# sjtuytc/UnboundedNeRFPytorch

Measured on AMD Instinct MI355X. Metric: Msamples/sec (Mip-360 garden-shaped 1920x1080x256 frame, FourierGrid render), higher is better.
Workload: dtype f32; 1 GPU; S1 1920x1080x256 G200 F3(P7) C12 rgbnet 39-128-128-3 f32 stepsize 1.31 thres 1e-4 white-noise grids; rays=2073600, samples_per_ray=256, chunks_per_frame=1, parallelism=1 GPU, step=ray generation + march + shade + un-tiling to image order; 3 frames in flight

## Files before the change

### unboundednerfpytorch_amd/csrc/ugrid_march.hip

```cpp
#include "ugrid_render.h"
#include "ugrid_rays.h"

__global__ void k_pack_bricks(const float *__restrict__ grid, int P, int C, int X, int Y, int Z, int H,
                              int CH, int coef, float *__restrict__ out, int64_t total) {
  for (int64_t o = (int64_t)blockIdx.x * blockDim.x + threadIdx.x; o < total;
       o += (int64_t)gridDim.x * blockDim.x) {
    int64_t q = o;
    int ch, c;
    if (H == 2) {
      const int qi = (int)(q % (8 * CH)); q /= (8 * CH);
      c = (qi >> 1) & 7;
      ch = (qi >> 4) * 2 + (qi & 1);
    } else {
      ch = (int)(q % CH); q /= CH;
      c = (int)(q % 8); q /= 8;
    }
    const int h = (int)(q % H); q /= H;
    const int k = (int)(q % (Z - 1)); q /= (Z - 1);
    const int j = (int)(q % (Y - 1)); q /= (Y - 1);
    const int i = (int)(q % (X - 1)); q /= (X - 1);
    const int l = (int)q;
    const int chan = h * CH + ch;
    float v = 0.f;
    if (chan < C) {
// ... 812 lines not shown
  UG_LAUNCH_CHECK();
  return 0;
}

extern "C" int ugrid_train_sample_compact_vox(int64_t n_rays, int32_t slots_per_ray, float act_shift, float interval, float thres,
                                              const float *scratch_pts, const float *scratch_density, const int32_t *scratch_step,
                                              const float *scratch_w, const float *scratch_T, const int32_t *count,
                                              const int64_t *offset_end, const int32_t *count2, const int64_t *offset_end2,
                                              const float *t_table, float *pts1, float *density1, float *weights1, float *T1,
                                              int32_t *pos2, float *pts2, float *density2, float *alpha2, float *weights2,
                                              int64_t *ray_id2, int64_t *step_id2, float *t2, uint8_t *inner2, ugrid_stream_t s) {
  if (n_rays <= 0) return 0;
  hipLaunchKernelGGL(k_train_compact2, dim3(ug_blocks(n_rays * UG_WAVE, 256)), dim3(256), 0, ST(s), n_rays, slots_per_ray, act_shift,
                     interval, thres, scratch_pts, scratch_density, scratch_step, scratch_w, scratch_T, count, offset_end, count2,
                     offset_end2, t_table, pts1, density1, weights1, T1, pos2, pts2, density2, alpha2, weights2, ray_id2, step_id2, t2,
                     inner2, ug_tl_devn.cap > 0 ? ug_tl_devn.cap : INT64_MAX);
  UG_LAUNCH_CHECK();
  return 0;
}

extern "C" int ugrid_train_sample_backward(int64_t n_rays, float act_shift, float interval, const float *density1,
                                           const float *weights1, const float *T1, const int32_t *pos2, const int32_t *count,
                                           const int64_t *offset_end, const float *alphainv_last, const float *g_weights2,
                                           const float *g_alphainv_last, const float *g_density2, float *g_density1,
                                           ugrid_stream_t s) {
  if (n_rays <= 0) return 0;
  hipLaunchKernelGGL(k_train_sample_bwd, dim3(ug_blocks(n_rays * UG_WAVE, 256)), dim3(256), 0, ST(s), n_rays, act_shift, interval,
                     density1, weights1, T1, pos2, count, offset_end, alphainv_last, g_weights2, g_alphainv_last, g_density2, g_density1);
  UG_LAUNCH_CHECK();
  return 0;
}

extern "C" int ugrid_train_compact(int64_t n_rays, int32_t n_samples, const float *scratch_pts, const float *scratch_density,
                                   const int32_t *scratch_step, const int32_t *count, const int64_t *offset_end,
                                   const float *t_table, float *pts, float *density, int64_t *ray_id, int64_t *step_id,
                                   float *t, ugrid_stream_t s) {
  if (n_rays <= 0) return 0;
  hipLaunchKernelGGL(k_train_compact, dim3(ug_blocks(n_rays * UG_WAVE, 256)), dim3(256), 0, ST(s), n_rays, n_samples,
                     scratch_pts, scratch_density, scratch_step, count, offset_end, t_table, pts, density, ray_id, step_id, t);
  UG_LAUNCH_CHECK();
  return 0;
}

template <class MarchTile>
__device__ __forceinline__ void ug_march_block(const ug_ws_view &ws, int64_t nblocks, MarchTile march) {
  const int64_t blk = ug_xcd_remap(blockIdx.x, nblocks);
  if (blk >= nblocks) return;
  const int64_t tile = blk * 4 + (threadIdx.x >> 6);
  if (tile >= ws.n_tiles) return;
  const int n = march(tile, ws.ent + tile * ws.cap, ws.slot + tile * ws.cap);
  if (ug_lane() == 0) ws.count[tile] = n;
}

struct ug_march_geom { ug_ws_view ws; int64_t nblocks; dim3 grid; };
static inline ug_march_geom ug_march_geometry(void *ws_mem, int64_t n_rays, int32_t S) {
  ug_march_geom g;
  g.ws = ug_ws_make(ws_mem, n_rays, S);
  g.nblocks = (g.ws.n_tiles + 3) / 4;
  g.grid = dim3((unsigned)(((g.nblocks + 7) / 8) * 8));
  return g;
}

template <int F, bool L2, int W>
__global__ void __launch_bounds__(256, W)
k_march(ug_march_args a, const float *__restrict__ rays_o, const float *__restrict__ rays_d,
        const float *__restrict__ t_table, const float *__restrict__ s_table,
        const float *__restrict__ bricks, float *__restrict__ alphainv_last, float *__restrict__ depth,
        ug_ws_view ws, int64_t nblocks) {
  ug_march_block(ws, nblocks, [&](int64_t tile, float4 *ent, uint8_t *slot) {
    return ug_march_tile<F, L2>(a, rays_o, rays_d, t_table, s_table, bricks, alphainv_last, depth, tile, ent, slot);
  });
}


template <bool L2>
__global__ void __launch_bounds__(256, 5)
k_march_dcvgo(ug_march_args a, ug_dc_args dc, const float *__restrict__ rays_o, const float *__restrict__ rays_d,
              const float *__restrict__ t_table, const float *__restrict__ s_table, const float *__restrict__ bricks,
              float *__restrict__ alphainv_last, float *__restrict__ depth, float *__restrict__ wsum_mid, ug_ws_view ws,
              int64_t nblocks) {
  ug_march_block(ws, nblocks, [&](int64_t tile, float4 *ent, uint8_t *slot) {
    return ug_march_tile<0, L2, true>(a, rays_o, rays_d, t_table, s_table, bricks, alphainv_last, depth, tile, ent, slot, dc, wsum_mid);
  });
}

__global__ void __launch_bounds__(256, 6)
k_march_dvgo(ug_march_args a, ug_dv_args dv, const float *__restrict__ rays_o, const float *__restrict__ rays_d,
             const float *__restrict__ bricks, float *__restrict__ alphainv_last, float *__restrict__ depth, ug_ws_view ws,
             int64_t nblocks) {
  ug_march_block(ws, nblocks, [&](int64_t tile, float4 *ent, uint8_t *slot) {
    return ug_march_tile_dvgo(a, dv, rays_o, rays_d, bricks, alphainv_last, depth, tile, ent, slot, a.S);
  });
}

__global__ void __launch_bounds__(256, 6)
k_march_mpi(ug_march_args a, ug_mpi_args mp, const float *__restrict__ rays_o, const float *__restrict__ rays_d,
            const float *__restrict__ bricks, const float *__restrict__ act_shift, float *__restrict__ alphainv_last,
            float *__restrict__ depth, ug_ws_view ws, int64_t nblocks) {
  __shared__ float shift[256];
  if ((int)threadIdx.x < mp.D) shift[threadIdx.x] = act_shift[threadIdx.x];
  __syncthreads();
  ug_march_block(ws, nblocks, [&](int64_t tile, float4 *ent, uint8_t *slot) {
    return ug_march_tile_mpi(a, mp, rays_o, rays_d, bricks, shift, alphainv_last, depth, tile, ent, slot);
  });
}

extern "C" int64_t ugrid_render_ws_bytes(int64_t n_rays, int32_t S) {
  const int64_t n_tiles = (n_rays + UG_WAVE - 1) / UG_WAVE, cap = (int64_t)UG_WAVE * S;
  return 256 + ug_align256(n_tiles * 4) + ug_align256(n_tiles * cap * 16) + ug_align256(n_tiles * cap);
}

static int ug_grid_query_any(bool cl, const float *grid, int P, int C, int X, int Y, int Z, const float *xyz,
                             const float *xyz_min, const float *xyz_max, int freq_num, int64_t n, float *out, hipStream_t st) {
  if (n <= 0) return 0;
  if (P != (freq_num > 0 ? 2 * freq_num + 1 : 1)) return (int)hipErrorInvalidValue;
  const int64_t nl = ug_launch_rows(n);
  if (cl)
    hipLaunchKernelGGL(HIP_KERNEL_NAME(k_grid_query<true>), dim3(ug_blocks(nl * C, 256)), dim3(256), 0, st, grid, P, C, X, Y, Z, xyz,
                       xyz_min, xyz_max, freq_num, n, out, ug_tl_devn.ptr);
  else
    hipLaunchKernelGGL(HIP_KERNEL_NAME(k_grid_query<false>), dim3(ug_blocks(nl, 256)), dim3(256), 0, st, grid, P, C, X, Y, Z, xyz,
                       xyz_min, xyz_max, freq_num, n, out, ug_tl_devn.ptr);
  UG_LAUNCH_CHECK();
// ... 51 lines not shown
                                            int Z, float *acc, ugrid_stream_t s) {
  if (n_rays <= 0 || n_samples <= 0) return 0;
  if (!rays_o || !rays_d || !xyz_min || !xyz_max || !acc || X < 1 || Y < 1 || Z < 1) return (int)hipErrorInvalidValue;
  hipLaunchKernelGGL(k_count_views_accumulate, dim3(ug_blocks(n_rays, 64)), dim3(64), 0, ST(s), rays_o, rays_d, n_rays, xyz_min, xyz_max,
                     near, far, stepdist, n_samples, X, Y, Z, acc);
  UG_LAUNCH_CHECK();
  return 0;
}

extern "C" int ugrid_count_views_commit(float *acc, float *count, int64_t n, ugrid_stream_t s) {
  if (n <= 0) return 0;
  if (!acc || !count) return (int)hipErrorInvalidValue;
  const int64_t blocks = ug_blocks(n, 256);
  hipLaunchKernelGGL(k_count_views_commit, dim3((unsigned)(blocks < 65536 ? blocks : 65536)), dim3(256), 0, ST(s), acc, count, n);
  UG_LAUNCH_CHECK();
  return 0;
}

static inline int ug_brick_ch(int C, int *H) {
  if (C == 1) { *H = 1; return 1; }
  *H = 2;
  return UG_CH(C);
}

extern "C" int64_t ugrid_brick_bytes(int P, int C, int X, int Y, int Z, int direct) {
  int H, CH = ug_brick_ch(C, &H);
  if (direct) { H = 1; CH = 4; }
  return (int64_t)P * (X - 1) * (Y - 1) * (Z - 1) * H * 8 * CH * (int64_t)sizeof(float);
}

extern "C" int ugrid_pack_bricks(const float *grid, int P, int C, int X, int Y, int Z, int direct,
                                 float *bricks, ugrid_stream_t s) {
  if (X < 2 || Y < 2 || Z < 2 || P < 1 || C < 1) return (int)hipErrorInvalidValue;
  int H, CH = ug_brick_ch(C, &H);
  if (direct) { H = 1; CH = 4; }
  const int64_t total = (int64_t)P * (X - 1) * (Y - 1) * (Z - 1) * H * 8 * CH;
  int64_t blocks = (total + 255) / 256;
  if (blocks > 256 * 64) blocks = 256 * 64;
  if (C == 12 && !direct) {
    if (P > 1 && (int64_t)(X - 1) * (Y - 1) * (Z - 1) * 384 >= ((int64_t)1 << 32)) return (int)hipErrorInvalidValue;
    hipLaunchKernelGGL(k_pack_quad, dim3((unsigned)blocks), dim3(256), 0, ST(s), grid, P, C, X, Y, Z, bricks, total);
    UG_LAUNCH_CHECK();
    return 0;
  }
  int coef = direct ? 0 : 1;
  hipLaunchKernelGGL(k_pack_bricks, dim3((unsigned)blocks), dim3(256), 0, ST(s), grid, P, C, X, Y, Z, H, CH,
                     coef, bricks, total);
  UG_LAUNCH_CHECK();
  return 0;
}

static int g_march_waves = 6;
extern "C" int ug_set_march_waves(int w) { if (w < 4 || w > 6) return 1; g_march_waves = w; return 0; }

template <int F, int W>
static int ug_march_launch_w(const ugrid_render_params *p, const ug_march_args &a, const float *rays_o,
                             const float *rays_d, const float *t_table, const float *s_table,
                             const float *bricks, float *alphainv_last, float *depth, const ug_march_geom &g,
                             hipStream_t st) {
  if (p->norm_l2)
    hipLaunchKernelGGL(HIP_KERNEL_NAME(k_march<F, true, W>), g.grid, dim3(256), 0, st, a, rays_o,
                       rays_d, t_table, s_table, bricks, alphainv_last, depth, g.ws, g.nblocks);
  else
    hipLaunchKernelGGL(HIP_KERNEL_NAME(k_march<F, false, W>), g.grid, dim3(256), 0, st, a, rays_o,
                       rays_d, t_table, s_table, bricks, alphainv_last, depth, g.ws, g.nblocks);
  UG_LAUNCH_CHECK();
  return 0;
}

template <int F>
static int ug_march_launch(const ugrid_render_params *p, const ug_march_args &a, const float *rays_o,
                           const float *rays_d, const float *t_table, const float *s_table,
                           const float *bricks, float *alphainv_last, float *depth, const ug_march_geom &g,
                           hipStream_t st) {
  switch (g_march_waves) {
    case 4: return ug_march_launch_w<F, 4>(p, a, rays_o, rays_d, t_table, s_table, bricks, alphainv_last, depth, g, st);
    case 6: return ug_march_launch_w<F, 6>(p, a, rays_o, rays_d, t_table, s_table, bricks, alphainv_last, depth, g, st);
    default: return ug_march_launch_w<F, 5>(p, a, rays_o, rays_d, t_table, s_table, bricks, alphainv_last, depth, g, st);
  }
}

extern "C" int ugrid_render_march(const ugrid_render_params *p, const float *rays_o, const float *rays_d,
                                  const float *t_table, const float *s_table, const float *density_bricks,
                                  float *alphainv_last, float *depth, void *ws_mem, ugrid_stream_t s) {
  if (p->n_rays <= 0) return 0;
  ug_march_args a;
  const int rc = ug_fill_march_args(p, a);
  if (rc) return rc;
  const ug_march_geom g = ug_march_geometry(ws_mem, p->n_rays, p->n_samples);
  switch (p->freq_num) {
    case 1: return ug_march_launch<1>(p, a, rays_o, rays_d, t_table, s_table, density_bricks, alphainv_last, depth, g, ST(s));
    case 2: return ug_march_launch<2>(p, a, rays_o, rays_d, t_table, s_table, density_bricks, alphainv_last, depth, g, ST(s));
    case 3: return ug_march_launch<3>(p, a, rays_o, rays_d, t_table, s_table, density_bricks, alphainv_last, depth, g, ST(s));
    case 4: return ug_march_launch<4>(p, a, rays_o, rays_d, t_table, s_table, density_bricks, alphainv_last, depth, g, ST(s));
    case 5: return ug_march_launch<5>(p, a, rays_o, rays_d, t_table, s_table, density_bricks, alphainv_last, depth, g, ST(s));
    default: return (int)hipErrorInvalidValue;
  }
}


extern "C" int ugrid_render_march_dcvgo(const ugrid_render_params *p, const ugrid_dcvgo_params *q, const float *rays_o,
                                        const float *rays_d, const float *t_table, const float *s_table,
                                        const float *density_bricks, float *alphainv_last, float *depth, float *wsum_mid,
                                        void *ws_mem, ugrid_stream_t s) {
  if (p->n_rays <= 0) return 0;
  if (p->freq_num != 0 || !q) return (int)hipErrorInvalidValue;
  ug_march_args a;
  ug_dc_args dc;
  int rc = ug_fill_mask_args(dc, q->mask, q->mask_x, q->mask_y, q->mask_z, q->xyz2ijk_scale, q->xyz2ijk_shift);
  if (!rc) rc = ug_fill_march_args(p, a);
  if (rc) return rc;
  dc.dist_thres = q->dist_thres;
  const ug_march_geom g = ug_march_geometry(ws_mem, p->n_rays, p->n_samples);
  if (p->norm_l2)
    hipLaunchKernelGGL(HIP_KERNEL_NAME(k_march_dcvgo<true>), g.grid, dim3(256), 0, ST(s), a, dc, rays_o, rays_d, t_table,
                       s_table, density_bricks, alphainv_last, depth, wsum_mid, g.ws, g.nblocks);
  else
    hipLaunchKernelGGL(HIP_KERNEL_NAME(k_march_dcvgo<false>), g.grid, dim3(256), 0, ST(s), a, dc, rays_o, rays_d, t_table,
                       s_table, density_bricks, alphainv_last, depth, wsum_mid, g.ws, g.nblocks);
  UG_LAUNCH_CHECK();
// ... 43 lines not shown
```

### unboundednerfpytorch_amd/csrc/ugrid_render.h

```cpp
#pragma once
#include "ugrid_common.h"
#include "ugrid_math.h"
#include <string.h>

#define UG_CH(C) (2 * (((C) + 3) / 4))
#define UG_MAX_F 5


typedef float f32x16 __attribute__((ext_vector_type(16)));

struct ug_vec3 { float x, y, z; };

__device__ __forceinline__ float ug_norm3_torch(float x, float y, float z) {
  return sqrtf(fmaf(z, z, fmaf(y, y, x * x)));
}

template <bool L2>
__device__ __forceinline__ ug_vec3 ug_contract(ug_vec3 p, float B, float A) {
  const float nrm = L2 ? ug_norm3_torch(p.x, p.y, p.z) : fmaxf(fabsf(p.x), fmaxf(fabsf(p.y), fabsf(p.z)));
  if (!(nrm <= 1.0f)) {
    const float sc = B - (1.0f / nrm) * A;
    p.x = p.x / nrm * sc;
    p.y = p.y / nrm * sc;
    p.z = p.z / nrm * sc;
// ... 478 lines not shown
  }
#pragma unroll
  for (int s = 0; s < CH; ++s) feat[s] = 0.f;
#pragma unroll
  for (int b0 = 0; b0 < P; b0 += NB) {
    float4 v[NB][2 * CH];
#pragma unroll
    for (int l = 0; l < NB; ++l)
      if (b0 + l < P) {
#pragma unroll
        for (int q = 0; q < 2 * CH; ++q) v[l][q] = c[b0 + l].rec[q];
      }
    __builtin_amdgcn_sched_barrier(0);
#pragma unroll
    for (int l = 0; l < NB; ++l)
      if (b0 + l < P) {
        const float tz = c[b0 + l].tz, ty = c[b0 + l].ty, tx = c[b0 + l].tx;
#pragma unroll
        for (int pr = 0; pr < CH / 2; ++pr) {
          const float4 q0 = v[l][4 * pr], q1 = v[l][4 * pr + 1], q2 = v[l][4 * pr + 2], q3 = v[l][4 * pr + 3];
          const float a00 = fmaf(q0.z, tz, q0.x), a01 = fmaf(q1.z, tz, q1.x);
          const float a10 = fmaf(q2.z, tz, q2.x), a11 = fmaf(q3.z, tz, q3.x);
          const float b00 = fmaf(q0.w, tz, q0.y), b01 = fmaf(q1.w, tz, q1.y);
          const float b10 = fmaf(q2.w, tz, q2.y), b11 = fmaf(q3.w, tz, q3.y);
          const float fa = fmaf(fmaf(a11, ty, a10), tx, fmaf(a01, ty, a00));
          const float fb = fmaf(fmaf(b11, ty, b10), tx, fmaf(b01, ty, b00));
          feat[2 * pr] = (b0 + l == 0) ? fa : feat[2 * pr] + fa;
          feat[2 * pr + 1] = (b0 + l == 0) ? fb : feat[2 * pr + 1] + fb;
        }
      }
  }
#pragma unroll
  for (int ch = 0; ch < CH; ++ch) feat[ch] = ug_div_r(feat[ch], (float)P, 1.0f / (float)P);
}

typedef float ug_f4 __attribute__((ext_vector_type(4)));
template <int IMM>
__device__ __forceinline__ ug_f4 ug_gload4(unsigned voff, const float *sbase) {
  ug_f4 r;
  asm volatile("global_load_dwordx4 %0, %1, %2 offset:%3" : "=v"(r) : "v"(voff), "s"(sbase), "n"(IMM) : "memory");
  return r;
}
template <int IMM>
__device__ __forceinline__ ug_f4 ug_gload4v(const char *vaddr) {
  ug_f4 r;
  asm volatile("global_load_dwordx4 %0, %1, off offset:%2" : "=v"(r) : "v"(vaddr), "n"(IMM) : "memory");
  return r;
}
template <int N>
__device__ __forceinline__ void ug_vmwait6(ug_f4 (&v)[6]) {
  asm volatile("s_waitcnt vmcnt(%6)" : "+v"(v[0]), "+v"(v[1]), "+v"(v[2]), "+v"(v[3]), "+v"(v[4]), "+v"(v[5]) : "n"(N));
}

template <int K>
__device__ __forceinline__ float ug_quad_bcast(float x) {
  return __int_as_float(__builtin_amdgcn_mov_dpp(__float_as_int(x), K * 0x55, 0xf, 0xf, true));
}

__device__ __forceinline__ void ug_quad_poly(const ug_f4 (&v)[6], float tx, float ty, float tz, bool first, float (&feat)[3]) {
#pragma unroll
  for (int c = 0; c < 3; ++c) {
    const ug_f4 lo = v[2 * c], hi = v[2 * c + 1];
    const float p00 = fmaf(lo.y, tz, lo.x), p01 = fmaf(lo.w, tz, lo.z);
    const float p10 = fmaf(hi.y, tz, hi.x), p11 = fmaf(hi.w, tz, hi.z);
    const float f = fmaf(fmaf(p11, ty, p10), tx, fmaf(p01, ty, p00));
    feat[c] = first ? f : feat[c] + f;
  }
}

struct ug_quad_axis { float lo, ex, ir, nm1, nm2; unsigned goff; };
__device__ __forceinline__ ug_quad_axis ug_quad_axis_of(const ug_shade_args &a, int g) {
  ug_quad_axis q;
  q.lo = g == 0 ? a.lox : (g == 1 ? a.loy : a.loz);
  q.ex = g == 0 ? a.ex : (g == 1 ? a.ey : a.ez);
  q.ir = g == 0 ? a.irx : (g == 1 ? a.iry : a.irz);
  const int n = g == 0 ? a.X : (g == 1 ? a.Y : a.Z);
  q.nm1 = (float)(n - 1); q.nm2 = (float)(n - 2);
  q.goff = (unsigned)g * 16u;
  return q;
}

template <int F, int NBL, int NR>
struct ug_gather_state {
  static constexpr int P = 2 * F + 1, NI = NR * P;
  unsigned off[NI];
  float tx[NI], ty[NI], tz[NI];
  ug_f4 v[NBL][6];
};

#define UG_ISSUE_ITEM(st_, i_)                                                                                     \
  if constexpr (F == 0) {      \
    const char *pa = (const char *)k0b + (uint64_t)st_.off[i_] * 384ull + (uint64_t)((ug_lane() & 3) * 16);        \
    st_.v[(i_) % NBL][0] = ug_gload4v<0>(pa);   st_.v[(i_) % NBL][1] = ug_gload4v<64>(pa);                          \
    st_.v[(i_) % NBL][2] = ug_gload4v<128>(pa); st_.v[(i_) % NBL][3] = ug_gload4v<192>(pa);                         \
    st_.v[(i_) % NBL][4] = ug_gload4v<256>(pa); st_.v[(i_) % NBL][5] = ug_gload4v<320>(pa);                         \
  } else {                                                                                                         \
    const float *lb = k0b + (int64_t)((i_) / NR) * lvl_floats;                                                     \
    st_.v[(i_) % NBL][0] = ug_gload4<0>(st_.off[i_], lb);   st_.v[(i_) % NBL][1] = ug_gload4<64>(st_.off[i_], lb);  \
    st_.v[(i_) % NBL][2] = ug_gload4<128>(st_.off[i_], lb); st_.v[(i_) % NBL][3] = ug_gload4<192>(st_.off[i_], lb); \
    st_.v[(i_) % NBL][4] = ug_gload4<256>(st_.off[i_], lb); st_.v[(i_) % NBL][5] = ug_gload4<320>(st_.off[i_], lb); \
  }

template <int F, int NBL, int NR>
__device__ __forceinline__ void ug_k0_gather_begin(const float *__restrict__ k0b, const ug_shade_args &a,
                                                   const ug_quad_axis &qa, const float (&p_g)[NR],
                                                   ug_gather_state<F, NBL, NR> &st) {
// ... 910 lines not shown
```

### unboundednerfpytorch_amd/csrc/ugrid_shade.hip

```cpp
#include "ugrid_render.h"
#include "ugrid_shade_pc.h"

extern "C" int ug_set_march_waves(int w);
extern "C" int ug_set_tv_xcd(int m);
extern "C" int ug_set_train_mlp(int m);
#define UG_PC12_NBL 3
static int g_shade_pc = 2;

__global__ void k_pack_mlp(const float *__restrict__ w0, const float *__restrict__ b0,
                           const float *__restrict__ w1, const float *__restrict__ b1,
                           const float *__restrict__ w2, const float *__restrict__ b2, int C, int n_emb,
                           ug_mlp_scales sc, float *__restrict__ out) {
  const ug_mlp_layout L = ug_mlp_lay(C, n_emb);
  const int mlp_in = C + n_emb;
  unsigned short *hx = (unsigned short *)(out + L.hxA1);
  const int n_hx = (L.hxB1 - L.hxA1) * 2;
  for (int i = blockIdx.x * blockDim.x + threadIdx.x; i < n_hx; i += gridDim.x * blockDim.x) {
    const int e = i & 7, lane = (i >> 3) & 63, u = i >> 9;
    const int part = u & 1, o = (u >> 1) & 3, step = u >> 3;
    float w = 0.f;
    if (step < L.KB1) {
      const int idx = 8 * step + e;
      const int col = idx < L.KL ? ug_in_col(idx, lane >> 5, C, n_emb, L.KL) : -1;
      if (col >= 0) w = w0[(32 * o + (lane & 31)) * mlp_in + col] * sc.sW1;
    } else {
      const int st = step - L.KB1;
      w = w1[(32 * o + (lane & 31)) * 128 + ug_feat_of(st >> 1, 8 * (st & 1) + e, lane >> 5)] * sc.sW2;
    }
    const _Float16 hh = (_Float16)w;
    const _Float16 ll = (_Float16)(w - (float)hh);
    hx[i] = __builtin_bit_cast(unsigned short, part == 0 ? hh : ll);
  }
  if (blockIdx.x == 0 && threadIdx.x < 4)
    out[L.hxS + threadIdx.x] = threadIdx.x == 0 ? sc.sX1 : (threadIdx.x == 1 ? sc.sX2 / (sc.sW1 * sc.sX1) : 0.f);
  unsigned short *bf = (unsigned short *)(out + L.bfA1);
  const int n_bf = (L.bfB1 - L.bfA1) * 2;
  for (int i = blockIdx.x * blockDim.x + threadIdx.x; i < n_bf; i += gridDim.x * blockDim.x) {
    const int e = i & 7, lane = (i >> 3) & 63, u = i >> 9;
    const int part = u % 3, o = (u / 3) & 3, step = u / 12;
    float w = 0.f;
    if (step < L.KB1) {
      const int idx = 8 * step + e;
      const int col = idx < L.KL ? ug_in_col(idx, lane >> 5, C, n_emb, L.KL) : -1;
      if (col >= 0) w = w0[(32 * o + (lane & 31)) * mlp_in + col];
    } else {
      const int st = step - L.KB1;
      w = w1[(32 * o + (lane & 31)) * 128 + ug_feat_of(st >> 1, 8 * (st & 1) + e, lane >> 5)];
    }
    const __bf16 hh = (__bf16)w;
    const float r1 = w - (float)hh;
    const __bf16 mm = (__bf16)r1;
    const __bf16 ll = (__bf16)(r1 - (float)mm);
    const __bf16 pick = part == 0 ? hh : (part == 1 ? mm : ll);
    bf[i] = __builtin_bit_cast(unsigned short, pick);
  }
  for (int i = blockIdx.x * blockDim.x + threadIdx.x; i < L.total; i += gridDim.x * blockDim.x) {
// ... 146 lines not shown
      finite = finite && std::isfinite(a);
      m1 = a > m1 ? a : m1;
      acc += a * (k < C ? fb : 1.0);
    }
    finite = finite && std::isfinite(acc);
    B1 = acc > B1 ? acc : B1;
  }
  for (size_t i = 0; i < (size_t)128 * 128; ++i) {
    const double a = std::fabs((double)h_w1[i]);
    finite = finite && std::isfinite(a);
    m2 = a > m2 ? a : m2;
  }
  const double B0 = fb > 1.0 ? fb : 1.0;
  ug_mlp_scales sc = {1.f, 1.f, 1.f, 1.f};
  bool ok = finite && k0_absmax > 0 && std::isfinite(fb) && std::isfinite(B1) && std::isfinite(m1) && std::isfinite(m2) &&
            m1 > 1e-30 && m2 > 1e-30 && B1 > 1e-30;
  if (ok) {
    sc.sX1 = ug_pow2_floor(32768.0 / B0);
    sc.sW1 = ug_pow2_floor(32768.0 / m1);
    sc.sX2 = ug_pow2_floor(32768.0 / B1);
    sc.sW2 = ug_pow2_floor(32768.0 / m2);
    const float lo = 1.0f / 1024.0f, hi = 1099511627776.0f;
    ok = sc.sX1 >= lo && sc.sX2 >= lo && sc.sW1 >= lo && sc.sW2 >= lo && sc.sX1 <= hi && sc.sX2 <= hi &&
         sc.sW1 <= hi && sc.sW2 <= hi;
    if (!ok) sc = {1.f, 1.f, 1.f, 1.f};
  }
  scales4[0] = sc.sX1; scales4[1] = sc.sW1; scales4[2] = sc.sX2; scales4[3] = sc.sW2;
  return ok ? 1 : 0;
}

extern "C" int ugrid_pack_mlp(const float *w0, const float *b0, const float *w1, const float *b1,
                              const float *w2, const float *b2, int32_t k0_channels, int32_t viewbase_pe,
                              int32_t width, float k0_absmax, float *packed, int32_t *best_mode,
                              ugrid_stream_t s) {
  if (width != 128) return (int)hipErrorInvalidValue;
  const int C = k0_channels, n_emb = 3 + 6 * (int)viewbase_pe, mlp_in = C + n_emb;
  std::vector<float> h0((size_t)128 * mlp_in), hb0(128), h1((size_t)128 * 128);
  UG_HIP(hipMemcpyAsync(h0.data(), w0, h0.size() * sizeof(float), hipMemcpyDeviceToHost, ST(s)));
  UG_HIP(hipMemcpyAsync(hb0.data(), b0, hb0.size() * sizeof(float), hipMemcpyDeviceToHost, ST(s)));
  UG_HIP(hipMemcpyAsync(h1.data(), w1, h1.size() * sizeof(float), hipMemcpyDeviceToHost, ST(s)));
  UG_HIP(hipStreamSynchronize(ST(s)));
  float sc4[4];
  const int ok = ugrid_mlp_fp16x2_scales(h0.data(), hb0.data(), h1.data(), k0_channels, viewbase_pe, k0_absmax, sc4);
  const ug_mlp_scales sc = {sc4[0], sc4[1], sc4[2], sc4[3]};
  hipLaunchKernelGGL(k_pack_mlp, dim3(64), dim3(256), 0, ST(s), w0, b0, w1, b1, w2, b2, C, n_emb, sc, packed);
  UG_LAUNCH_CHECK();
  if (best_mode) *best_mode = (ok && viewbase_pe <= 4) ? UGRID_MLP_FP16X2 : UGRID_MLP_BF16X3;
  return 0;
}

extern "C" int ugrid_tune(const char *key, int value) {
  if (!key) return (int)hipErrorInvalidValue;
  if (!strcmp(key, "march_waves")) return ug_set_march_waves(value) ? (int)hipErrorInvalidValue : 0;
  if (!strcmp(key, "tv_xcd")) return ug_set_tv_xcd(value) ? (int)hipErrorInvalidValue : 0;
  if (!strcmp(key, "train_mlp")) return ug_set_train_mlp(value) ? (int)hipErrorInvalidValue : 0;
  if (!strcmp(key, "shade_pc") && value >= 0 && value <= 2) { g_shade_pc = value; return 0; }
  return (int)hipErrorInvalidValue;
}

template <int F, int C, int PE, int NW, int BF>
static int ug_shade_launch_nw(const ug_shade_args &a, const float *viewdirs, const float *k0b, const float *mlp,
                              ug_ws_view ws, float *rgb, int32_t *counter, hipStream_t st) {
  const int lds_bytes = ug_shade_lds_bytes<C, PE, BF, NW>();
  UG_SET_DYN_LDS((k_shade_mlp<F, C, PE, NW, BF>), lds_bytes);
  UG_ZERO_WORDS(counter, 8, st);
  int64_t wgs = (ws.n_tiles + NW - 1) / NW;
  if (wgs > 256) wgs = 256;
  wgs = (wgs + 7) / 8 * 8;
  hipLaunchKernelGGL(HIP_KERNEL_NAME(k_shade_mlp<F, C, PE, NW, BF>), dim3((unsigned)wgs), dim3(NW * 64), lds_bytes, st, a,
                     viewdirs, k0b, mlp, ws, rgb, counter);
  UG_LAUNCH_CHECK();
  return 0;
}


template <int F, int PE, int NPAIR, int SLOTS, int NBL, int MODE, bool ROLL = false>
static int ug_shade_pc_launch(const ug_shade_args &a, const float *viewdirs, const float *k0b, const float *mlp,
                              ug_ws_view ws, float *rgb, int32_t *counter, hipStream_t st) {
  const int lds_bytes = ug_pc_lds_bytes<PE, NPAIR, SLOTS>();
  if (lds_bytes > 160 * 1024) return (int)hipErrorInvalidValue;
  UG_SET_DYN_LDS((k_shade_pc<F, PE, NPAIR, SLOTS, NBL, MODE, ROLL>), lds_bytes);
  UG_ZERO_WORDS(counter, 8, st);
  int64_t wgs = (ws.n_tiles + NPAIR - 1) / NPAIR;
  if (wgs > 256) wgs = 256;
  wgs = (wgs + 7) / 8 * 8;
  hipLaunchKernelGGL(HIP_KERNEL_NAME(k_shade_pc<F, PE, NPAIR, SLOTS, NBL, MODE, ROLL>), dim3((unsigned)wgs), dim3(NPAIR * 128), lds_bytes, st,
                     a, viewdirs, k0b, mlp, ws, rgb, counter);
  UG_LAUNCH_CHECK();
  return 0;
}

template <int F, int C, int PE>
static int ug_shade_launch(const ug_shade_args &a, const float *viewdirs, const float *k0b, const float *mlp,
                           ug_ws_view ws, float *rgb, int32_t *counter, int mlp_mode, hipStream_t st) {
  if constexpr (PE > 4) {
    if (mlp_mode == UGRID_MLP_FP16X2) return (int)hipErrorInvalidValue;
  }
  if constexpr (C == 12 && PE <= 4) {
    if constexpr (F <= 3) {
      if (mlp_mode == UGRID_MLP_FP16X2 && g_shade_pc >= 2)
        return ug_shade_pc_launch<F, PE, 6, 2, UG_PC12_NBL, 1>(a, viewdirs, k0b, mlp, ws, rgb, counter, st);
    } else {
      if (mlp_mode == UGRID_MLP_FP16X2 && g_shade_pc >= 2)
        return ug_shade_pc_launch<F, PE, 6, 2, UG_PC12_NBL, 1, true>(a, viewdirs, k0b, mlp, ws, rgb, counter, st);
    }
    if (mlp_mode == UGRID_MLP_FP16X2 && g_shade_pc >= 1)
// ... 52 lines not shown
```

Measured before the change: 64940 Msamples/s.

## Add software-pipelined march kernel that prefetches brick loads across levels and samples

Adds a new march kernel, on by default, that uses a K-deep register ring of in-flight brick loads across the Fourier levels and issues the next sample's loads while the current sample's levels are still being consumed, using explicit vmcnt waits and scheduling barriers. Ray data and positions are staged in LDS, and t/s table values are read with scalar loads. The goal is to hide global memory latency in the density march. The cost is more registers and LDS per thread, which can lower occupancy, and a large amount of hand-scheduled inline asm that is fragile.

Measured after the change: 64030 Msamples/s. 0.986x the previous value.

```diff
diff --git a/unboundednerfpytorch_amd/csrc/ugrid_march.hip b/unboundednerfpytorch_amd/csrc/ugrid_march.hip
--- a/unboundednerfpytorch_amd/csrc/ugrid_march.hip
+++ b/unboundednerfpytorch_amd/csrc/ugrid_march.hip
@@ -888,6 +888,16 @@
   if (ug_lane() == 0) ws.count[tile] = n;
 }
 
+template <class MarchTile>
+__device__ __forceinline__ void ug_march_block_uniform(const ug_ws_view &ws, int64_t nblocks, MarchTile march) {
+  const int64_t blk = ug_xcd_remap(blockIdx.x, nblocks);
+  if (blk >= nblocks) return;
+  const int64_t tile = blk * 4 + __builtin_amdgcn_readfirstlane((int)(threadIdx.x >> 6));
+  if (tile >= ws.n_tiles) return;
+  const int n = march(tile, ws.ent + tile * ws.cap, ws.slot + tile * ws.cap);
+  if (ug_lane() == 0) ws.count[tile] = n;
+}
+
 struct ug_march_geom { ug_ws_view ws; int64_t nblocks; dim3 grid; };
 static inline ug_march_geom ug_march_geometry(void *ws_mem, int64_t n_rays, int32_t S) {
   ug_march_geom g;
@@ -905,6 +915,17 @@
         ug_ws_view ws, int64_t nblocks) {
   ug_march_block(ws, nblocks, [&](int64_t tile, float4 *ent, uint8_t *slot) {
     return ug_march_tile<F, L2>(a, rays_o, rays_d, t_table, s_table, bricks, alphainv_last, depth, tile, ent, slot);
+  });
+}
+
+template <int F, bool L2, int W>
+__global__ void __launch_bounds__(256, W)
+k_march_pipe(ug_march_args a, const float *__restrict__ rays_o, const float *__restrict__ rays_d,
+             const float *__restrict__ t_table, const float *__restrict__ s_table,
+             const float *__restrict__ bricks, float *__restrict__ alphainv_last, float *__restrict__ depth,
+             ug_ws_view ws, int64_t nblocks) {
+  ug_march_block_uniform(ws, nblocks, [&](int64_t tile, float4 *ent, uint8_t *slot) {
+    return ug_march_tile_pipe<F, L2>(a, rays_o, rays_d, t_table, s_table, bricks, alphainv_last, depth, tile, ent, slot);
   });
 }
 
@@ -1062,20 +1083,38 @@
 
 static int g_march_waves = 6;
 extern "C" int ug_set_march_waves(int w) { if (w < 4 || w > 6) return 1; g_march_waves = w; return 0; }
+static int g_march_pipe = 1;
+extern "C" int ug_set_march_pipe(int m) { if (m < 0 || m > 1) return 1; g_march_pipe = m; return 0; }
+
+template <int F, int W, bool PIPE>
+static int ug_march_launch_wp(const ugrid_render_params *p, const ug_march_args &a, const float *rays_o,
+                             const float *rays_d, const float *t_table, const float *s_table,
+                             const float *bricks, float *alphainv_last, float *depth, const ug_march_geom &g,
+                             hipStream_t st) {
+  if constexpr (PIPE) {
+    if (p->norm_l2)
+      hipLaunchKernelGGL(HIP_KERNEL_NAME(k_march_pipe<F, true, W>), g.grid, dim3(256), 0, st, a, rays_o,
+                         rays_d, t_table, s_table, bricks, alphainv_last, depth, g.ws, g.nblocks);
+    else
+      hipLaunchKernelGGL(HIP_KERNEL_NAME(k_march_pipe<F, false, W>), g.grid, dim3(256), 0, st, a, rays_o,
+                         rays_d, t_table, s_table, bricks, alphainv_last, depth, g.ws, g.nblocks);
+  } else if (p->norm_l2)
+    hipLaunchKernelGGL(HIP_KERNEL_NAME(k_march<F, true, W>), g.grid, dim3(256), 0, st, a, rays_o,
+                       rays_d, t_table, s_table, bricks, alphainv_last, depth, g.ws, g.nblocks);
+  else
+    hipLaunchKernelGGL(HIP_KERNEL_NAME(k_march<F, false, W>), g.grid, dim3(256), 0, st, a, rays_o,
+                       rays_d, t_table, s_table, bricks, alphainv_last, depth, g.ws, g.nblocks);
+  UG_LAUNCH_CHECK();
+  return 0;
+}
 
 template <int F, int W>
 static int ug_march_launch_w(const ugrid_render_params *p, const ug_march_args &a, const float *rays_o,
                              const float *rays_d, const float *t_table, const float *s_table,
                              const float *bricks, float *alphainv_last, float *depth, const ug_march_geom &g,
                              hipStream_t st) {
-  if (p->norm_l2)
-    hipLaunchKernelGGL(HIP_KERNEL_NAME(k_march<F, true, W>), g.grid, dim3(256), 0, st, a, rays_o,
-                       rays_d, t_table, s_table, bricks, alphainv_last, depth, g.ws, g.nblocks);
-  else
-    hipLaunchKernelGGL(HIP_KERNEL_NAME(k_march<F, false, W>), g.grid, dim3(256), 0, st, a, rays_o,
-                       rays_d, t_table, s_table, bricks, alphainv_last, depth, g.ws, g.nblocks);
-  UG_LAUNCH_CHECK();
-  return 0;
+  if (g_march_pipe) return ug_march_launch_wp<F, W, true>(p, a, rays_o, rays_d, t_table, s_table, bricks, alphainv_last, depth, g, st);
+  return ug_march_launch_wp<F, W, false>(p, a, rays_o, rays_d, t_table, s_table, bricks, alphainv_last, depth, g, st);
 }
 
 template <int F>
diff --git a/unboundednerfpytorch_amd/csrc/ugrid_render.h b/unboundednerfpytorch_amd/csrc/ugrid_render.h
--- a/unboundednerfpytorch_amd/csrc/ugrid_render.h
+++ b/unboundednerfpytorch_amd/csrc/ugrid_render.h
@@ -554,6 +554,238 @@
   asm volatile("s_waitcnt vmcnt(%6)" : "+v"(v[0]), "+v"(v[1]), "+v"(v[2]), "+v"(v[3]), "+v"(v[4]), "+v"(v[5]) : "n"(N));
 }
 
+template <int N>
+__device__ __forceinline__ void ug_vmwait2(ug_f4 &lo, ug_f4 &hi) {
+  asm volatile("s_waitcnt vmcnt(%2)" : "+v"(lo), "+v"(hi) : "n"(N));
+}
+
+#ifndef UG_MARCH_PIPE_K
+#define UG_MARCH_PIPE_K 4
+#endif
+constexpr int ug_mp_last(int P, int K, int s) { return s + K * ((P - 1 - s) / K); }
+constexpr int ug_mp_when(int P, int K, int s) {
+  int e = P - K - 1 > 0 ? P - K - 1 : 0;
+  for (int i = 0; i <= s; ++i) e = ug_mp_last(P, K, i) > e ? ug_mp_last(P, K, i) : e;
+  return e;
+}
+constexpr int ug_mp_after(int P, int K, int l) {
+  int n = (l + K - 1 < P - 1 ? l + K - 1 : P - 1) - l;
+  for (int s = 0; s < K; ++s) n += ug_mp_when(P, K, s) < l ? 1 : 0;
+  return n;
+}
+
+__device__ __forceinline__ float ug_sload(const float *p) {
+  float v;
+  asm volatile("s_load_dword %0, %1, 0x0" : "=s"(v) : "s"(p) : "memory");
+  return v;
+}
+__device__ __forceinline__ void ug_swait(float &v) { asm volatile("s_waitcnt lgkmcnt(0)" : "+s"(v)); }
+
+__device__ __forceinline__ float ug_uniformf(float v) {
+  return __uint_as_float(__builtin_amdgcn_readfirstlane(__float_as_uint(v)));
+}
+struct ug_mp_grid { float xm1, xm2, ym1, ym2, zm1, zm2; unsigned zrow, off_max; };
+__device__ __forceinline__ void ug_mp_axis(float c, float nm1, float nm2, float &cellf, float &whi) {
+  const float ix = fmaf(c, 0.5f, 0.5f) * nm1;
+  cellf = __builtin_amdgcn_fmed3f(floorf(ix), 0.0f, nm2);
+  whi = ix - cellf;
+}
+
+struct ug_mp_pt { float ux, uy, uz; };
+
+template <int K>
+struct ug_mp_ring {
+  ug_f4 lo[K], hi[K];
+  float tx[K], ty[K], tz[K];
+  float cx, cy, cz;
+};
+
+template <bool L2>
+__device__ __forceinline__ ug_mp_pt ug_mp_point(const ug_march_args &a, const float *ray_lds, float *pos_lds, float t) {
+  const float ox = ray_lds[0], oy = ray_lds[256], oz = ray_lds[512], dx = ray_lds[768], dy = ray_lds[1024], dz = ray_lds[1280];
+  float px = ox + dx * t, py = oy + dy * t, pz = oz + dz * t;
+  const float nrm = L2 ? ug_norm3_torch(px, py, pz) : fmaxf(fabsf(px), fmaxf(fabsf(py), fabsf(pz)));
+  if (!(nrm <= 1.0f)) {
+    const float rn = ug_rcp_refined(nrm);
+    const float sc = a.B - rn * a.A;
+    px = ug_div_r(px, nrm, rn) * sc;
+    py = ug_div_r(py, nrm, rn) * sc;
+    pz = ug_div_r(pz, nrm, rn) * sc;
+  }
+  ug_mp_pt q;
+  pos_lds[0] = px; pos_lds[256] = py; pos_lds[512] = pz;
+  ug_normalise(a, px, py, pz, q.ux, q.uy, q.uz);
+  return q;
+}
+
+template <int K, int L>
+__device__ __forceinline__ void ug_mp_issue(const ug_mp_grid &g, const char *__restrict__ bkb, size_t lvl_bytes,
+                                            const ug_mp_pt &q, ug_mp_ring<K> &r) {
+  constexpr int s = L % K;
+  float cx, cy, cz;
+  if constexpr (L == 0) {
+    cx = q.ux; cy = q.uy; cz = q.uz;
+  } else if constexpr ((L & 1) != 0) {
+    constexpr int k = (L - 1) / 2;
+    if constexpr (k == 0) {
+      ug_sincos_small(q.ux, &cx, &r.cx);
+      __builtin_amdgcn_sched_barrier(0);
+      ug_sincos_small(q.uy, &cy, &r.cy);
+      __builtin_amdgcn_sched_barrier(0);
+      ug_sincos_small(q.uz, &cz, &r.cz);
+    } else {
+      const float f = (float)(1 << k);
+      ug_sincos(f * q.ux, &cx, &r.cx);
+      __builtin_amdgcn_sched_barrier(0);
+      ug_sincos(f * q.uy, &cy, &r.cy);
+      __builtin_amdgcn_sched_barrier(0);
+      ug_sincos(f * q.uz, &cz, &r.cz);
+    }
+    asm volatile("" : "+v"(r.cx), "+v"(r.cy), "+v"(r.cz));
+    __builtin_amdgcn_sched_barrier(0);
+  } else {
+    cx = r.cx; cy = r.cy; cz = r.cz;
+  }
+  float cfx, cfy, cfz;
+  ug_mp_axis(cx, g.xm1, g.xm2, cfx, r.tx[s]);
+  ug_mp_axis(cy, g.ym1, g.ym2, cfy, r.ty[s]);
+  ug_mp_axis(cz, g.zm1, g.zm2, cfz, r.tz[s]);
+  const unsigned row = (unsigned)fmaf(cfx, g.ym1, cfy);
+  unsigned off = __umul24(row, g.zrow) + ((unsigned)(int)cfz << 5);
+  off = off < g.off_max ? off : g.off_max;
+  asm volatile("" : "+v"(r.tx[s]), "+v"(r.ty[s]), "+v"(r.tz[s]));
+  const float *lb = (const float *)(bkb + (size_t)L * lvl_bytes);
+  r.lo[s] = ug_gload4<0>(off, lb);
+  r.hi[s] = ug_gload4<16>(off, lb);
+  __builtin_amdgcn_sched_barrier(0);
+}
+
+template <int K, int P, int L, int S_>
+__device__ __forceinline__ void ug_mp_issue_next(const ug_mp_grid &g, const char *__restrict__ bkb, size_t lvl_bytes,
+                                                 const ug_mp_pt &nxt, ug_mp_ring<K> &r) {
+  if constexpr (S_ < K) {
+    if constexpr (ug_mp_when(P, K, S_) == L) ug_mp_issue<K, S_>(g, bkb, lvl_bytes, nxt, r);
+    ug_mp_issue_next<K, P, L, S_ + 1>(g, bkb, lvl_bytes, nxt, r);
+  }
+}
+
+template <int K, int S_>
+__device__ __forceinline__ void ug_mp_prime(const ug_mp_grid &g, const char *__restrict__ bkb, size_t lvl_bytes,
+                                            const ug_mp_pt &q, ug_mp_ring<K> &r) {
+  if constexpr (S_ < K) {
+    ug_mp_issue<K, S_>(g, bkb, lvl_bytes, q, r);
+    ug_mp_prime<K, S_ + 1>(g, bkb, lvl_bytes, q, r);
+  }
+}
+
+template <bool L2, int K, int P, int L>
+__device__ __forceinline__ void ug_mp_levels(const ug_march_args &a, const ug_mp_grid &g, const char *__restrict__ bkb, size_t lvl_bytes,
+                                             const float *ray_lds, float *pos_next, float t_next, const ug_mp_pt &cur,
+                                             ug_mp_pt &nxt, ug_mp_ring<K> &r, float &dens) {
+  if constexpr (L < P) {
+    constexpr int s = L % K;
+    if constexpr (L == ug_mp_when(P, K, 0)) nxt = ug_mp_point<L2>(a, ray_lds, pos_next, t_next);
+    ug_vmwait2<2 * ug_mp_after(P, K, L)>(r.lo[s], r.hi[s]);
+    const ug_f4 v0 = r.lo[s], v1 = r.hi[s];
+    const float tz = r.tz[s], ty = r.ty[s], tx = r.tx[s];
+    const float p00 = fmaf(v0.y, tz, v0.x), p01 = fmaf(v0.w, tz, v0.z);
+    const float p10 = fmaf(v1.y, tz, v1.x), p11 = fmaf(v1.w, tz, v1.z);
+    const float d = fmaf(fmaf(p11, ty, p10), tx, fmaf(p01, ty, p00));
+    dens = (L == 0) ? d : dens + d;
+    asm volatile("" :: "v"(dens));
+    __builtin_amdgcn_sched_barrier(0);
+    if constexpr (L + K < P) ug_mp_issue<K, L + K>(g, bkb, lvl_bytes, cur, r);
+    ug_mp_issue_next<K, P, L, 0>(g, bkb, lvl_bytes, nxt, r);
+    __builtin_amdgcn_sched_barrier(0);
+    ug_mp_levels<L2, K, P, L + 1>(a, g, bkb, lvl_bytes, ray_lds, pos_next, t_next, cur, nxt, r, dens);
+  }
+}
+
+template <int F, bool L2>
+__device__ __forceinline__ int ug_march_tile_pipe(const ug_march_args &a, const float *__restrict__ rays_o,
+                                                  const float *__restrict__ rays_d, const float *__restrict__ t_table,
+                                                  const float *__restrict__ s_table, const float *__restrict__ bricks,
+                                                  float *__restrict__ alphainv_last, float *__restrict__ depth,
+                                                  int64_t tile, float4 *__restrict__ ent, uint8_t *__restrict__ slot) {
+  constexpr int P = 2 * F + 1;
+  constexpr int K = UG_MARCH_PIPE_K < P ? UG_MARCH_PIPE_K : P;
+  const int lane = ug_lane();
+  const int64_t ray0 = tile * UG_WAVE;
+  const bool valid = lane < (a.n_rays - ray0 < UG_WAVE ? (int)(a.n_rays - ray0) : UG_WAVE);
+
+  float ox = 0.f, oy = 0.f, oz = 0.f, dx = 0.f, dy = 0.f, dz = 1.f;
+  if (valid) {
+    const float *ro = rays_o + 3 * ray0, *rd = rays_d + 3 * ray0;
+    const float rox = ro[3 * lane], roy = ro[3 * lane + 1], roz = ro[3 * lane + 2];
+    const float rdx = rd[3 * lane], rdy = rd[3 * lane + 1], rdz = rd[3 * lane + 2];
+    ox = (rox - a.cx) / a.rx; oy = (roy - a.cy) / a.ry; oz = (roz - a.cz) / a.rz;
+    const float dn = ug_norm3_torch(rdx, rdy, rdz);
+    dx = rdx / dn; dy = rdy / dn; dz = rdz / dn;
+  }
+
+  const size_t lvl_bytes = (size_t)(a.X - 1) * (a.Y - 1) * (a.Z - 1) * 32;
+  ug_mp_grid g;
+  g.xm1 = ug_uniformf((float)(a.X - 1)); g.xm2 = ug_uniformf((float)(a.X - 2));
+  g.ym1 = ug_uniformf((float)(a.Y - 1)); g.ym2 = ug_uniformf((float)(a.Y - 2));
+  g.zm1 = ug_uniformf((float)(a.Z - 1)); g.zm2 = ug_uniformf((float)(a.Z - 2));
+  g.zrow = (unsigned)(a.Z - 1) << 5;
+  g.off_max = (unsigned)(lvl_bytes - 32);
+  const char *__restrict__ bkb = (const char *)bricks;
+
+  float T = 1.f, dsum = 0.f;
+  bool done = !valid;
+  int nsurv = 0;
+
+  __shared__ float mp_lds[12 * 256];
+  float *const lds = mp_lds + threadIdx.x;
+  lds[0] = ox; lds[256] = oy; lds[512] = oz; lds[768] = dx; lds[1024] = dy; lds[1280] = dz;
+  float *const pos_lds = lds + 6 * 256;
+
+  ug_mp_ring<K> ring;
+  ug_mp_pt cur = ug_mp_point<L2>(a, lds, pos_lds, t_table[0]);
+  __builtin_amdgcn_sched_barrier(0);
+  ug_mp_prime<K, 0>(g, bkb, lvl_bytes, cur, ring);
+  __builtin_amdgcn_sched_barrier(0);
+
+  for (int j = 0; j < a.S; ++j) {
+    if (__ballot(!done) == 0ull) break;
+    float t_next = ug_sload(t_table + (j + 1 < a.S ? j + 1 : a.S - 1)), s_j = ug_sload(s_table + j);
+    ug_swait(t_next); ug_swait(s_j);
+    ug_mp_pt nxt;
+    float dens;
+    float *const pos_cur = pos_lds + (j & 1) * 768, *const pos_next = pos_lds + ((j + 1) & 1) * 768;
+    ug_mp_levels<L2, K, P, 0>(a, g, bkb, lvl_bytes, lds, pos_next, t_next, cur, nxt, ring, dens);
+    bool surv = false;
+    float w = 0.f;
+    if (!done) {
+      dens = ug_div_r(dens, (float)P, 1.0f / (float)P);
+      const float xs = dens + a.shift;
+      const float alpha = ug_alpha(xs, a.interval);
+      if (alpha > a.thres) {
+        w = T * alpha;
+        T = (float)((double)T * (1. - (double)alpha));
+        if (w > a.thres) {
+          surv = true;
+          dsum += w * s_j;
+        }
+        if ((double)T < 1e-3) done = true;
+      }
+    }
+    float px = 0.f, py = 0.f, pz = 0.f;
+    if (surv) { px = pos_cur[0]; py = pos_cur[256]; pz = pos_cur[512]; }
+    ug_append_survivors(surv, px, py, pz, w, lane, ent, slot, nsurv);
+    cur = nxt;
+  }
+  __builtin_amdgcn_sched_barrier(0);
+  asm volatile("s_waitcnt vmcnt(0)" ::: "memory");
+  __builtin_amdgcn_sched_barrier(0);
+  if (valid) {
+    (alphainv_last + ray0)[lane] = T;
+    (depth + ray0)[lane] = dsum;
+  }
+  return nsurv;
+}
+
 template <int K>
 __device__ __forceinline__ float ug_quad_bcast(float x) {
   return __int_as_float(__builtin_amdgcn_mov_dpp(__float_as_int(x), K * 0x55, 0xf, 0xf, true));
diff --git a/unboundednerfpytorch_amd/csrc/ugrid_shade.hip b/unboundednerfpytorch_amd/csrc/ugrid_shade.hip
--- a/unboundednerfpytorch_amd/csrc/ugrid_shade.hip
+++ b/unboundednerfpytorch_amd/csrc/ugrid_shade.hip
@@ -2,6 +2,7 @@
 #include "ugrid_shade_pc.h"
 
 extern "C" int ug_set_march_waves(int w);
+extern "C" int ug_set_march_pipe(int m);
 extern "C" int ug_set_tv_xcd(int m);
 extern "C" int ug_set_train_mlp(int m);
 #define UG_PC12_NBL 3
@@ -254,6 +255,7 @@
 extern "C" int ugrid_tune(const char *key, int value) {
   if (!key) return (int)hipErrorInvalidValue;
   if (!strcmp(key, "march_waves")) return ug_set_march_waves(value) ? (int)hipErrorInvalidValue : 0;
+  if (!strcmp(key, "march_pipe")) return ug_set_march_pipe(value) ? (int)hipErrorInvalidValue : 0;
   if (!strcmp(key, "tv_xcd")) return ug_set_tv_xcd(value) ? (int)hipErrorInvalidValue : 0;
   if (!strcmp(key, "train_mlp")) return ug_set_train_mlp(value) ? (int)hipErrorInvalidValue : 0;
   if (!strcmp(key, "shade_pc") && value >= 0 && value <= 2) { g_shade_pc = value; return 0; }
```
